# Ntropy86/review-recommender

Hardware: AMD Instinct MI355X
Metric: queries/sec at top-k=100 (hybrid alpha=0.5) (higher is better)
Workload: dtype f32; 1 GPU; hybrid BM25+dense alpha=0.5 top-k=100 pool=150, 10000000 products x 384 fp32, BM25 ~40 tokens/doc vocab 200000 (327073593 postings on rank 0, 11164874 postings per query), batches of 256 queries; query_sets=4, docs=10000000, docs_per_gpu=10000000, batch=256, k=100, pool=150, parallelism=single GPU: no collective

## Files before the change

review-recommender_amd/csrc/rr_dense.hip:

```cpp
#include <stdlib.h>

#include "rr_common.h"
#include "rr_dense.h"
#include "rr_x3.h"

#define RR_SEL_THREADS 1024
#define RR_SEL_GCAP 4096
#define RR_SEL_CCAP 12288
#define RR_SEL_SORTCAP 8192
#define RR_SEL_RCAP 8192
#define RR_SEL_LCAP 4096

template <int NF>
__device__ __forceinline__ void rr_load_rows(f32x4 (&dst)[NF], const f32x4* __restrict__ mat,
                                             int64_t row, int64_t n_rows, int sub) {
    row = row < n_rows ? row : n_rows - 1;
    const f32x4* p = mat + row * (int64_t)(NF * 16) + sub;
#pragma unroll
    for (int i = 0; i < NF; ++i) dst[i] = __builtin_nontemporal_load(p + 16 * i);
}

template <int NF, int NB, bool FROM_LDS>
__device__ __forceinline__ void rr_dot_rows(const f32x4 (&x)[NF], const f32x4 (&qreg)[NF],
                                            const f32x4 (*qs)[NF * 16], int sub, int it,
// ... 376 lines not shown
    uint32_t n_cand = counters[1];

    if (n_cand > RR_SEL_SORTCAP) {
        uint64_t prefix = 0, mask = 0;
        uint32_t k = (uint32_t)pool;
        for (int shift = 56; shift >= 0; shift -= 8) {
            if (tid < 256) hist[tid] = 0;
            __syncthreads();
            for (int64_t i = tid; i < n_slots; i += RR_SEL_THREADS) {
                const int64_t t = all_tiles ? (i >> 6) : (int64_t)glist[i >> 6];
                const int64_t row = t * 64 + (i & 63);
                if (row < n_rows) {
                    const uint64_t key = ((uint64_t)rr_f2key(score_at(row)) << 32) |
                                         (uint64_t)(0xFFFFFFFFu - (uint32_t)row);
                    if ((key & mask) == prefix) atomicAdd(&hist[(key >> shift) & 255u], 1u);
                }
            }
            __syncthreads();
            rr_pick_bin(hist, wsum, sel, k);
            prefix |= (uint64_t)sel[0] << shift;
            mask |= (uint64_t)255u << shift;
            k -= sel[1];
            __syncthreads();
        }
        if (tid == 0) counters[1] = 0;
        __syncthreads();
        for (int64_t i = tid; i < n_slots; i += RR_SEL_THREADS) {
            const int64_t t = all_tiles ? (i >> 6) : (int64_t)glist[i >> 6];
            const int64_t row = t * 64 + (i & 63);
            if (row < n_rows) {
                const uint64_t key = ((uint64_t)rr_f2key(score_at(row)) << 32) |
                                     (uint64_t)(0xFFFFFFFFu - (uint32_t)row);
                if (key >= prefix) {
                    const uint32_t slot = atomicAdd(&counters[1], 1u);
                    if (slot < RR_SEL_SORTCAP) cand[slot] = key;
                }
            }
        }
        __syncthreads();
        n_cand = counters[1] < RR_SEL_SORTCAP ? counters[1] : RR_SEL_SORTCAP;
    }

    if (n_cand > RR_SEL_SORTCAP) n_cand = RR_SEL_SORTCAP;
    int n_sort = 1;
    while (n_sort < (int)n_cand) n_sort <<= 1;
    for (int i = tid; i < n_sort; i += RR_SEL_THREADS)
        if (i >= (int)n_cand) cand[i] = 0;
    rr_bitonic_desc(cand, n_sort);
}

#define RR_SEL_RK 8
template <int RK>
__device__ uint32_t rr_kth_largest_reg(const uint32_t (&r)[RR_SEL_RK], int n_mine, uint32_t k,
                                       uint32_t (*cnt)[3][16], int& phase, int max_steps) {
    const int tid = threadIdx.x;
    const int ln = tid & 63;
    uint32_t mx = 0, mn = 0xFFFFFFFFu, nz = 0;
#pragma unroll
    for (int j = 0; j < RK; ++j) {
        const bool live = j < n_mine && r[j] != 0u;
        if (j < n_mine) mx = r[j] > mx ? r[j] : mx;
        if (live) mn = r[j] < mn ? r[j] : mn;
        nz += (uint32_t)__popcll(__ballot(live));
    }
#pragma unroll
    for (int m = 32; m >= 1; m >>= 1) {
        const uint32_t a = __shfl_xor(mx, m, 64), b = __shfl_xor(mn, m, 64);
        mx = a > mx ? a : mx;
        mn = b < mn ? b : mn;
    }
    if (ln == 0) {
        cnt[phase][0][tid >> 6] = mx;
        cnt[phase][1][tid >> 6] = mn;
        cnt[phase][2][tid >> 6] = nz;
    }
    __syncthreads();
    uint32_t nz_all = 0;
    for (int w = 0; w < 16; ++w) {
        mx = cnt[phase][0][w] > mx ? cnt[phase][0][w] : mx;
        mn = cnt[phase][1][w] < mn ? cnt[phase][1][w] : mn;
        nz_all += cnt[phase][2][w];
    }
    if (nz_all < k) mn = 0u;
    phase ^= 1;
    if (mx == mn) return mx;
    int bit = 31 - __clz(mx ^ mn);
    uint32_t prefix = (bit == 31) ? 0u : (mx >> (bit + 1)) << (bit + 1);
    for (int step = 0; bit >= 0 && step < max_steps; ++step) {
        const int lo = bit >= 1 ? bit - 1 : 0;
        const bool two = bit >= 1;
        const uint32_t t1 = prefix | (1u << lo);
        const uint32_t t2 = prefix | (1u << bit);
        const uint32_t t3 = prefix | (1u << bit) | (1u << lo);
        uint32_t c1 = 0, c2 = 0, c3 = 0;
#pragma unroll
        for (int j = 0; j < RK; ++j) {
            const bool have = j < n_mine;
            c1 += (uint32_t)__popcll(__ballot(have && r[j] >= t1));
            c2 += (uint32_t)__popcll(__ballot(have && r[j] >= t2));
            c3 += (uint32_t)__popcll(__ballot(have && r[j] >= t3));
        }
        if (ln == 0) {
            cnt[phase][0][tid >> 6] = c1;
            cnt[phase][1][tid >> 6] = c2;
            cnt[phase][2][tid >> 6] = c3;
        }
        __syncthreads();
        int v = ln < 48 ? (int)(&cnt[phase][0][0])[ln] : 0;
        v += __builtin_amdgcn_update_dpp(0, v, 0xB1, 0xF, 0xF, true);
        v += __builtin_amdgcn_update_dpp(0, v, 0x4E, 0xF, 0xF, true);
        v += __builtin_amdgcn_update_dpp(0, v, 0x141, 0xF, 0xF, true);
        v += __builtin_amdgcn_update_dpp(0, v, 0x140, 0xF, 0xF, true);
        const uint32_t s1 = (uint32_t)__builtin_amdgcn_readlane(v, 0);
        const uint32_t s2 = (uint32_t)__builtin_amdgcn_readlane(v, 16);
        const uint32_t s3 = (uint32_t)__builtin_amdgcn_readlane(v, 32);
        phase ^= 1;
        if (two) {
            if (s3 >= k) prefix = t3;
            else if (s2 >= k) prefix = t2;
            else if (s1 >= k) prefix = t1;
        } else if (s2 >= k) {
            prefix = t2;
        }
        bit = lo - 1;
    }
    return prefix;
}

__device__ void rr_rank_sort_desc(const uint64_t* keys, int n, uint64_t* out) {
    const int tid = threadIdx.x;
    uint64_t mine = 0;
    int rank = 0;
    if (tid < n) {
        mine = keys[tid];
        for (int j = 0; j < n; ++j) rank += keys[j] > mine ? 1 : 0;
    }
    __syncthreads();
    if (tid < n) out[rank] = mine;
    __syncthreads();
}

template <typename GroupKeyAt>
__device__ uint32_t rr_sel_open_groups(GroupKeyAt group_key_at, int ng, int pool, uint32_t (*cnt)[3][16],
                                       int& phase, uint32_t* counters, uint32_t* list2,
                                       float eps2 = -1.f, uint32_t* open_key = nullptr, uint32_t thr_floor = 0u) {
    const int tid = threadIdx.x;
    uint32_t r[RR_SEL_RK];
    int n_mine = 0;
#pragma unroll
    for (int j = 0; j < RR_SEL_RK; ++j) {
        const int i = tid + j * RR_SEL_THREADS;
        r[j] = i < ng ? group_key_at(i) : 0u;
        n_mine += i < ng ? 1 : 0;
    }
    uint32_t tau = 1u;
    if (ng > pool) {
        if (ng <= 1 * RR_SEL_THREADS) tau = rr_kth_largest_reg<1>(r, n_mine, (uint32_t)pool, cnt, phase, 7);
        else if (ng <= 2 * RR_SEL_THREADS) tau = rr_kth_largest_reg<2>(r, n_mine, (uint32_t)pool, cnt, phase, 7);
        else if (ng <= 4 * RR_SEL_THREADS) tau = rr_kth_largest_reg<4>(r, n_mine, (uint32_t)pool, cnt, phase, 7);
        else tau = rr_kth_largest_reg<8>(r, n_mine, (uint32_t)pool, cnt, phase, 7);
    }
    if (tau == 0u) tau = 1u;
    uint32_t thr = tau;
    if (eps2 >= 0.f) {
        thr = rr_f2key(rr_key2f(tau) - eps2);
        if (thr == 0u) thr = 1u;
        if (thr_floor > thr) thr = thr_floor;
        if (open_key) *open_key = thr;
    }
#pragma unroll
    for (int j = 0; j < RR_SEL_RK; ++j) {
        if (j < n_mine && r[j] >= thr) {
            const uint32_t slot = atomicAdd(&counters[0], 1u);
            if (slot < RR_SEL_LCAP) list2[slot] = (uint32_t)(tid + j * RR_SEL_THREADS);
        }
    }
    __syncthreads();
    return tau;
}

__global__ __launch_bounds__(RR_SEL_THREADS) void rr_select(
    rr_scan_geom G, const float* __restrict__ sims, const float* __restrict__ gmax,
    const uint32_t* __restrict__ smax, int pool, int64_t row_offset,
    int64_t* __restrict__ out_rows, float* __restrict__ out_scores, int32_t* __restrict__ dbg,
    const int32_t* __restrict__ only_if, int n_total, int64_t sims_slice, int64_t gmax_slice, int64_t smax_slice,
    const int32_t* __restrict__ qlist, int32_t* __restrict__ clear_flags) {
    if (qlist) {
        if ((int)blockIdx.x >= qlist[0]) return;
        const int qo = qlist[1 + blockIdx.x] - (int)blockIdx.x;
        out_rows += (int64_t)qo * pool; out_scores += (int64_t)qo * pool; dbg += qo * 16;
        if (threadIdx.x == 0) clear_flags[qo + (int)blockIdx.x] = 0;
    }
    if (gridDim.y > 1) {
        const int y = blockIdx.y;
        if (64 * y + (int)blockIdx.x >= n_total) return;
        only_if += 64 * y;
        out_rows += (int64_t)64 * y * pool; out_scores += (int64_t)64 * y * pool; dbg += 64 * y * 16;
        sims += y * sims_slice; gmax += y * gmax_slice; smax += y * smax_slice;
    }
    if (only_if && !only_if[blockIdx.x]) return;
    __shared__ uint32_t hist[256];
    __shared__ uint32_t wsum[4];
    __shared__ uint32_t cnt[2][3][16];
    __shared__ uint32_t sel[2];
    __shared__ uint32_t counters[4];
    __shared__ uint32_t list2[RR_SEL_LCAP];
    __shared__ uint32_t list1[RR_SEL_GCAP];
    __shared__ uint64_t cand[RR_SEL_CCAP];

    const int tid = threadIdx.x;
    const int q = blockIdx.x;
    const int QS = G.qs;
    auto score_at = [&](int64_t row) -> float {
        return QS ? sims[((row >> 4) * QS + q) * 16 + (row & 15)] : sims[(int64_t)q * G.n_pad + row];
    };
    auto tile_max_at = [&](int64_t t) -> float {
        return QS ? gmax[t * QS + q] : gmax[(int64_t)q * G.n_tiles + t];
    };
    auto group_key_at = [&](int i) -> uint32_t {
        return QS ? smax[(int64_t)i * QS + q] : smax[(int64_t)q * G.n_waves + i];
    };
    const int64_t n_rows = G.n_rows, n_tiles = G.n_tiles;
    int phase = 0;
    long long stamp[8];
    int n_stamp = 0;
#define RR_STAMP() do { if (n_stamp < 8) stamp[n_stamp++] = clock64(); } while (0)
    RR_STAMP();
    const int ng = G.n_waves;
    bool fast = ng <= RR_SEL_RK * RR_SEL_THREADS;

    if (tid < 4) counters[tid] = 0;
    __syncthreads();

    if (fast) {
        const uint32_t tau = rr_sel_open_groups(group_key_at, ng, pool, cnt, phase, counters, list2);
        RR_STAMP();
        if (counters[0] > RR_SEL_LCAP) fast = false;

        if (fast) {
            const int C = (int)G.tiles_per_wave;
            const int64_t n2 = (int64_t)counters[0] * C;
            for (int64_t i = tid; i < n2; i += RR_SEL_THREADS) {
                const int64_t t = (int64_t)list2[i / C] * C + (i % C);
                if (t < n_tiles && rr_f2key(tile_max_at(t)) >= tau) {
                    const uint32_t slot = atomicAdd(&counters[1], 1u);
                    if (slot < RR_SEL_GCAP) list1[slot] = (uint32_t)t;
                }
            }
            __syncthreads();
            if (counters[1] > RR_SEL_GCAP) fast = false;
        }
        RR_STAMP();
        if (fast) {
            const int n1 = (int)counters[1] * 64;
            for (int i = tid; i < n1; i += RR_SEL_THREADS) {
                const uint32_t row = list1[i >> 6] * 64u + (uint32_t)(i & 63);
                if ((int64_t)row < n_rows) {
                    const uint32_t key = rr_f2key(score_at(row));
                    if (key >= tau) {
                        const uint32_t slot = atomicAdd(&counters[2], 1u);
                        if (slot < RR_SEL_CCAP / 2)
                            cand[slot] = ((uint64_t)key << 32) | (uint64_t)(0xFFFFFFFFu - row);
                    }
                }
            }
            __syncthreads();
            RR_STAMP();
            const uint32_t n_cand = counters[2];
            if (n_cand > RR_SEL_CCAP / 2 || n_cand < (uint32_t)pool) {
                fast = false;
            } else if (n_cand <= RR_SEL_THREADS) {
                rr_rank_sort_desc(cand, (int)n_cand, cand + RR_SEL_CCAP / 2);
                for (int i = tid; i < pool; i += RR_SEL_THREADS) cand[i] = cand[RR_SEL_CCAP / 2 + i];
                __syncthreads();
            } else {
                int n_sort = 1;
                while (n_sort < (int)n_cand) n_sort <<= 1;
                for (int i = tid; i < n_sort; i += RR_SEL_THREADS)
                    if (i >= (int)n_cand) cand[i] = 0;
                rr_bitonic_desc(cand, n_sort);
            }
        }
    }
    RR_STAMP();
    if (tid == 0) {
        dbg[q * 16 + 0] = fast ? 1 : 0;
        dbg[q * 16 + 1] = (int32_t)counters[0];
        dbg[q * 16 + 2] = (int32_t)counters[1];
        dbg[q * 16 + 3] = (int32_t)counters[2];
        for (int i = 1; i < 8; ++i) dbg[q * 16 + 3 + i] = i < n_stamp ? (int32_t)(stamp[i] - stamp[i - 1]) : -1;
    }
    if (!fast) {
        __syncthreads();
        rr_select_slow(score_at, tile_max_at, n_rows, n_tiles, pool, hist, wsum, sel, counters, list1, cand);
    }
    for (int i = tid; i < pool; i += RR_SEL_THREADS) {
        const uint64_t key = cand[i];
        const uint32_t row = 0xFFFFFFFFu - (uint32_t)(key & 0xFFFFFFFFu);
        out_rows[(int64_t)q * pool + i] = (int64_t)row + row_offset;
        out_scores[(int64_t)q * pool + i] = rr_key2f((uint32_t)(key >> 32));
    }
}

__global__ __launch_bounds__(RR_SEL_THREADS) void rr_select_mtiles(
    rr_scan_geom G, const float* __restrict__ mmax, const uint32_t* __restrict__ smax, int pool,
    uint32_t* __restrict__ out_mtiles, int32_t* __restrict__ out_count, uint32_t* __restrict__ out_tau,
    int32_t* __restrict__ fb, int32_t* __restrict__ dbg, const float* __restrict__ eps,
    const float* __restrict__ sigma, int nq_a, int nq_b, int64_t mmax_set_stride, int64_t smax_set_stride,
    const float* __restrict__ floor) {
    __shared__ uint32_t cnt[2][3][16];
    __shared__ uint32_t counters[4];
    __shared__ uint32_t list2[RR_SEL_LCAP];
    const int tid = threadIdx.x;
    const int Q = blockIdx.x;
    const int set = (nq_b > 0 && Q >= nq_a) ? 1 : 0;
    const int q = set ? Q - nq_a : Q;
    const int nq_set = set ? nq_b : nq_a;
    mmax += set * mmax_set_stride;
    smax += set * smax_set_stride;
    if (eps) eps += set * RR_FLT_MAXQ;
    if (sigma) sigma += set * RR_FLT_MAXQ;
    out_mtiles += (int64_t)(Q - q) * RR_X3_MCAP;
    out_count += Q - q; out_tau += Q - q; fb += Q - q; dbg += (Q - q) * 16;
    const int QS = G.qs;
    auto group_key_at = [&](int i) -> uint32_t { return smax[(int64_t)i * QS + q]; };
    const int gpw = G.gpw > 1 ? G.gpw : 1;
    const int ng = G.n_waves * gpw;
    int phase = 0;
    const long long c0 = clock64();
    long long c1 = c0, c2 = c0;
    if (tid < 4) counters[tid] = 0;
    __syncthreads();
    bool ok = ng <= RR_SEL_RK * RR_SEL_THREADS && ng > pool;
    uint32_t tau = 1u;
    uint32_t open = 1u;
    if (ok) {
        const float e = eps ? eps[q] : -1.f;
        if (eps && !(e >= 0.f && e < 3.0e38f)) ok = false;
        if (ok) {
            const float fl = (floor && eps) ? floor[Q] - 1.05f * e : -INFINITY;
            if (fl > -3.0e38f) {
                open = rr_f2key(fl);
                if (open == 0u) open = 1u;
                for (int i = tid; i < ng; i += RR_SEL_THREADS) {
                    if (group_key_at(i) >= open) {
                        const uint32_t slot = atomicAdd(&counters[0], 1u);
                        if (slot < RR_SEL_LCAP) list2[slot] = (uint32_t)i;
                    }
                }
                __syncthreads();
                tau = rr_f2key(floor[Q]);
                if (counters[0] > RR_SEL_LCAP) {
                    __syncthreads();
                    if (tid == 0) counters[0] = 0;
                    __syncthreads();
                    const uint32_t floor_open = open, floor_tau = tau;
                    tau = rr_sel_open_groups(group_key_at, ng, pool, cnt, phase, counters, list2, 2.05f * e, &open, floor_open);
                    tau = rr_f2key(rr_key2f(tau) - 1.02f * e);
                    if (floor_tau > tau) tau = floor_tau;
                }
            } else {
                tau = rr_sel_open_groups(group_key_at, ng, pool, cnt, phase, counters, list2, eps ? 2.05f * e : -1.f, &open, 0u);
                if (!eps) open = tau;
                else tau = rr_f2key(rr_key2f(tau) - 1.02f * e);
            }
            if (tau == 0u) tau = 1u;
            if (counters[0] > RR_SEL_LCAP) ok = false;
        }
    }
    c1 = clock64();
    if (ok) {
        const int C = (int)G.tiles_per_group;
        const int64_t n2 = (int64_t)counters[0] * C;
        const f32x4* mm4 = reinterpret_cast<const f32x4*>(mmax);
        if (G.mm_pairs == 3) {
            constexpr int U = 4;
            const float step = rr_flt_gap_step(eps, nq_set);
            const float openf = open <= 0x007FFFFFu ? -INFINITY : rr_key2f(open);
            if (sigma && !(sigma[q] <= openf)) ok = false;
            const int n2i = (int)n2;
            for (int i0 = tid; i0 < n2i; i0 += U * RR_SEL_THREADS) {
                int64_t tt[U];
                uint32_t w0[U], w1[U];
#pragma unroll
                for (int u = 0; u < U; ++u) {
                    const int i = i0 + u * RR_SEL_THREADS;
                    tt[u] = -1;
                    if (i < n2i) {
                        const int g = (int)list2[i / C], k = g % gpw, j = i % C;
                        const int64_t in_run = (int64_t)k * C + j;
                        const int64_t t = (int64_t)(g / gpw) * G.tiles_per_wave + in_run;
                        if (in_run < G.tiles_per_wave && t < G.n_tiles) tt[u] = t;
                    }
                    const int64_t ts = tt[u] < 0 ? 0 : tt[u];
                    w0[u] = reinterpret_cast<const uint32_t*>(mmax)[(2 * ts) * QS + q];
                    w1[u] = reinterpret_cast<const uint32_t*>(mmax)[(2 * ts + 1) * QS + q];
                }
#pragma unroll
                for (int u = 0; u < U; ++u) {
                    if (tt[u] < 0) continue;
#pragma unroll
                    for (int half = 0; half < 2; ++half) {
                        const uint32_t w = half ? w1[u] : w0[u];
                        const float mx = __uint_as_float(w << 16);
                        if (!(mx >= openf)) continue;
#pragma unroll
                        for (int g = 0; g < 4; ++g) {
                            const uint32_t code = (w >> (16 + 4 * g)) & 15u;
                            const float bound = mx - rr_flt_gap_steps(code) * step;
                            if (bound >= openf) {
                                const uint32_t slot = atomicAdd(&counters[1], 1u);
                                if (slot < RR_X3_MCAP) out_mtiles[(int64_t)q * RR_X3_MCAP + slot] = (uint32_t)(tt[u] * 8 + 4 * half + g);
                            }
                        }
                    }
                }
            }
        } else
        for (int64_t i = tid; i < n2; i += RR_SEL_THREADS) {
            const int g = (int)list2[i / C], k = g % gpw, j = (int)(i % C);
            const int64_t in_run = (int64_t)k * C + j;
            const int64_t t = (int64_t)(g / gpw) * G.tiles_per_wave + in_run;
            if (in_run >= G.tiles_per_wave || t >= G.n_tiles) continue;
            float v[4];
            if (G.mm_pairs) {
                const float2 m0 = reinterpret_cast<const float2*>(mmax)[(2 * t) * QS + q];
                const float2 m1 = reinterpret_cast<const float2*>(mmax)[(2 * t + 1) * QS + q];
                v[0] = m0.x, v[1] = m0.y, v[2] = m1.x, v[3] = m1.y;
            } else {
                const f32x4 m = mm4[t * QS + q];
                v[0] = m.x, v[1] = m.y, v[2] = m.z, v[3] = m.w;
            }
#pragma unroll
            for (int sub = 0; sub < 4; ++sub) {
                if (rr_f2key(v[sub]) >= open) {
                    const uint32_t slot = atomicAdd(&counters[1], 1u);
                    if (slot < RR_X3_MCAP) out_mtiles[(int64_t)q * RR_X3_MCAP + slot] = (uint32_t)(t * 4 + sub);
                }
            }
        }
        __syncthreads();
        if (counters[1] > RR_X3_MCAP) ok = false;
    }
    c2 = clock64();
    if (tid == 0) {
        out_count[q] = ok ? (int32_t)counters[1] : 0;
        out_tau[q] = tau;
        fb[q] = ok ? 0 : 1;
        dbg[q * 16 + 0] = ok ? 2 : 0;
        dbg[q * 16 + 1] = (int32_t)counters[0];
        dbg[q * 16 + 2] = (int32_t)counters[1];
        dbg[q * 16 + 3] = 0;
        dbg[q * 16 + 4] = (int32_t)(c1 - c0);
        dbg[q * 16 + 5] = (int32_t)(c2 - c1);
        for (int i = 6; i < 16; ++i) dbg[q * 16 + i] = -1;
#ifdef RR_DEBUG_HARNESS
        dbg[q * 16 + 6] = (int32_t)open;
#endif
    }
}

template <int RCAP>
__global__ __launch_bounds__(RR_SEL_THREADS) void rr_select_rescored(
    rr_scan_geom G, const uint32_t* __restrict__ mtiles, const int32_t* __restrict__ count,
    const uint32_t* __restrict__ tau_of, const float* __restrict__ sc, int pool, int64_t row_offset,
    int64_t* __restrict__ out_rows, float* __restrict__ out_scores, int32_t* __restrict__ fb,
    int32_t* __restrict__ dbg, int floor_mode) {
    __shared__ uint32_t counters[2];
    __shared__ uint64_t cand[RCAP];
    const int tid = threadIdx.x;
    const int q = blockIdx.x;
    if (fb[q]) return;
    if (tid < 2) counters[tid] = 0;
    __syncthreads();
    const uint32_t tau = tau_of[q];
    const int sh = G.mm_pairs == 3 ? 3 : 4;
    const int n1 = count[q] << sh;
    const bool all_rows = floor_mode && (uint32_t)n1 <= RCAP / 2;
    for (int i = tid; i < n1 && !all_rows; i += RR_SEL_THREADS) {
        const int64_t at = (int64_t)q * RR_X3_MCAP + (i >> sh);
        const int r = i & ((1 << sh) - 1);
        const uint32_t row = (mtiles[at] << sh) + (uint32_t)r;
        if ((int64_t)row < G.n_rows) {
            const uint32_t key = rr_f2key(sc[(at << sh) + r]);
            if (key >= tau) {
                const uint32_t slot = atomicAdd(&counters[0], 1u);
                if (slot < RCAP / 2) cand[slot] = ((uint64_t)key << 32) | (uint64_t)(0xFFFFFFFFu - row);
            }
        }
    }
    __syncthreads();
    uint32_t n_cand = counters[0];
    if (all_rows || (floor_mode && n_cand < (uint32_t)pool && (uint32_t)n1 <= RCAP / 2)) {
        __syncthreads();
        if (tid == 0) counters[0] = 0;
        __syncthreads();
        for (int i = tid; i < n1; i += RR_SEL_THREADS) {
            const int64_t at = (int64_t)q * RR_X3_MCAP + (i >> sh);
            const int r = i & ((1 << sh) - 1);
            const uint32_t row = (mtiles[at] << sh) + (uint32_t)r;
            if ((int64_t)row < G.n_rows) {
                const uint32_t key = rr_f2key(sc[(at << sh) + r]);
                const uint32_t slot = atomicAdd(&counters[0], 1u);
                if (slot < RCAP / 2) cand[slot] = ((uint64_t)key << 32) | (uint64_t)(0xFFFFFFFFu - row);
            }
        }
        __syncthreads();
        n_cand = counters[0];
    }
    if (tid == 0) dbg[q * 16 + 3] = (int32_t)n_cand;
    if (n_cand > RCAP / 2 || n_cand < (uint32_t)pool) {
        if (tid == 0) {
            fb[q] = 1;
            dbg[q * 16 + 0] = 0;
        }
        return;
    }
    if (n_cand <= RR_SEL_THREADS) {
        rr_rank_sort_desc(cand, (int)n_cand, cand + RCAP / 2);
        for (int i = tid; i < pool; i += RR_SEL_THREADS) cand[i] = cand[RCAP / 2 + i];
        __syncthreads();
    } else {
        int n_sort = 1;
        while (n_sort < (int)n_cand) n_sort <<= 1;
        for (int i = tid; i < n_sort; i += RR_SEL_THREADS)
            if (i >= (int)n_cand) cand[i] = 0;
        rr_bitonic_desc(cand, n_sort);
    }
    for (int i = tid; i < pool; i += RR_SEL_THREADS) {
        const uint64_t key = cand[i];
        const uint32_t row = 0xFFFFFFFFu - (uint32_t)(key & 0xFFFFFFFFu);
        out_rows[(int64_t)q * pool + i] = (int64_t)row + row_offset;
        out_scores[(int64_t)q * pool + i] = rr_key2f((uint32_t)(key >> 32));
    }
}

rr_x3_scratch rr_x3_scratch_of(const rr_index* ix) {
    rr_x3_scratch s;
    char* p = static_cast<char*>(ix->d_x3);
    s.mtiles = reinterpret_cast<uint32_t*>(p);  p += sizeof(uint32_t) * RR_SEL_MAXQ * RR_X3_MCAP;
    s.count = reinterpret_cast<int32_t*>(p);    p += sizeof(int32_t) * RR_SEL_MAXQ;
    s.tau = reinterpret_cast<uint32_t*>(p);     p += sizeof(uint32_t) * RR_SEL_MAXQ;
    s.fb = reinterpret_cast<int32_t*>(p);       p += sizeof(int32_t) * RR_SEL_MAXQ;
    p += sizeof(float) * RR_SEL_MAXQ;
    s.eps = ix->d_eps;
    s.sc = reinterpret_cast<float*>(p);
    return s;
}
size_t rr_x3_scratch_bytes() {
    return sizeof(uint32_t) * RR_SEL_MAXQ * RR_X3_MCAP + 4 * sizeof(int32_t) * RR_SEL_MAXQ +
           sizeof(float) * (size_t)RR_SEL_MAXQ * RR_X3_MCAP * 16;
}
void rr_launch_select_mtiles(rr_index* ix, const rr_scan_geom& G, int nq, int pool, hipStream_t st, const float* eps,
                             const float* sigma, int nq_b, int64_t mmax_set_stride, int64_t smax_set_stride,
                             const float* floor) {
    const rr_x3_scratch s = rr_x3_scratch_of(ix);
    hipLaunchKernelGGL(rr_select_mtiles, dim3(nq + nq_b), dim3(RR_SEL_THREADS), 0, st, G, ix->d_gmax, ix->d_smax, pool,
                       s.mtiles, s.count, s.tau, s.fb, ix->d_sel_trace, eps, sigma, nq, nq_b, mmax_set_stride,
                       smax_set_stride, floor);
}
void rr_launch_select_rescored(rr_index* ix, const rr_scan_geom& G, int nq, int pool, int64_t* d_rows,
                               float* d_scores, hipStream_t st, bool floor_mode) {
    const rr_x3_scratch s = rr_x3_scratch_of(ix);
    if (pool <= 512)
        hipLaunchKernelGGL((rr_select_rescored<RR_SEL_RCAP>), dim3(nq), dim3(RR_SEL_THREADS), 0, st, G, s.mtiles, s.count, s.tau,
                           s.sc, pool, ix->row_offset, d_rows, d_scores, s.fb, ix->d_sel_trace, floor_mode ? 1 : 0);
    else
        hipLaunchKernelGGL((rr_select_rescored<RR_SEL_CCAP>), dim3(nq), dim3(RR_SEL_THREADS), 0, st, G, s.mtiles, s.count, s.tau,
                           s.sc, pool, ix->row_offset, d_rows, d_scores, s.fb, ix->d_sel_trace, floor_mode ? 1 : 0);
}

__global__ __launch_bounds__(RR_SEL_THREADS) void rr_group_kth(rr_scan_geom G, const uint32_t* __restrict__ smax, int kth,
                                                               const float* __restrict__ eps, float* __restrict__ bound,
                                                               int nq_a, int nq_b, int64_t smax_set_stride) {
    __shared__ uint32_t cnt[2][3][16];
    const int tid = threadIdx.x;
    const int Q = blockIdx.x;
    const int set = (nq_b > 0 && Q >= nq_a) ? 1 : 0;
    const int q = set ? Q - nq_a : Q;
    smax += set * smax_set_stride;
    eps += set * RR_FLT_MAXQ;
    const int QS = G.qs;
    const int gpw = G.gpw > 1 ? G.gpw : 1;
    const int ng = G.n_waves * gpw;
    int phase = 0;
    float out = -INFINITY;
    if (ng > kth && ng <= RR_SEL_RK * RR_SEL_THREADS) {
        uint32_t r[RR_SEL_RK];
        int n_mine = 0;
#pragma unroll
        for (int j = 0; j < RR_SEL_RK; ++j) {
            const int i = tid + j * RR_SEL_THREADS;
            r[j] = i < ng ? smax[(int64_t)i * QS + q] : 0u;
            n_mine += i < ng ? 1 : 0;
        }
        uint32_t tau;
        if (ng <= 1 * RR_SEL_THREADS) tau = rr_kth_largest_reg<1>(r, n_mine, (uint32_t)kth, cnt, phase, 7);
        else if (ng <= 2 * RR_SEL_THREADS) tau = rr_kth_largest_reg<2>(r, n_mine, (uint32_t)kth, cnt, phase, 7);
        else if (ng <= 4 * RR_SEL_THREADS) tau = rr_kth_largest_reg<4>(r, n_mine, (uint32_t)kth, cnt, phase, 7);
        else tau = rr_kth_largest_reg<8>(r, n_mine, (uint32_t)kth, cnt, phase, 7);
        const float e = eps[q];
        if (tau > 0x007FFFFFu && e >= 0.f && e < 3.0e38f) out = rr_key2f(tau) - 1.01f * e;
        if (!(out == out)) out = -INFINITY;
    }
    if (tid == 0) bound[Q] = out;
}
void rr_launch_group_kth(rr_index* ix, const rr_scan_geom& G, int nq_a, int nq_b, int kth, const float* eps, float* d_bound,
                         int64_t smax_set_stride, hipStream_t st) {
    hipLaunchKernelGGL(rr_group_kth, dim3(nq_a + nq_b), dim3(RR_SEL_THREADS), 0, st, G, ix->d_smax, kth, eps, d_bound, nq_a,
                       nq_b, smax_set_stride);
}

__global__ void rr_l2norm_f32(float* __restrict__ mat, int64_t n_rows, int dim_pad, float eps) {
    const int lane = threadIdx.x & 63;
    const int64_t row = (int64_t)blockIdx.x * (blockDim.x >> 6) + (threadIdx.x >> 6);
    if (row >= n_rows) return;
    float* p = mat + row * dim_pad;
    float ss = 0.f;
    for (int i = lane; i < dim_pad; i += 64) ss = __builtin_fmaf(p[i], p[i], ss);
#pragma unroll
    for (int m = 32; m >= 1; m >>= 1) ss += __shfl_xor(ss, m, 64);
    const float nrm = fmaxf(sqrtf(ss), eps);
    for (int i = lane; i < dim_pad; i += 64) p[i] = p[i] / nrm;
}

static int rr_ensure_maxima(rr_index* ix, int nq) {
    const size_t nm = nq >= RR_MFMA_MAXQ ? RR_FLT_MAXQ : nq;
    if (ix->maxima_q >= (int)nm) return RR_OK;
    const int64_t n_tiles = rr_round_up(ix->n_rows, 64) / 64;
    if (ix->d_gmax) hipFree(ix->d_gmax);
    if (ix->d_smax) hipFree(ix->d_smax);
    ix->d_gmax = nullptr;
    ix->d_smax = nullptr;
    ix->maxima_q = 0;
    const size_t groups_cap = (size_t)RR_MAX_SCAN_WAVES;
    const size_t gmax_words = nm * n_tiles * 4 + (size_t)RR_MAX_SCAN_WAVES * RR_FLT_MAXQ;
    RR_HIP_TRY(hipMalloc(&ix->d_gmax, sizeof(float) * gmax_words));
    RR_HIP_TRY(hipMemsetD32Async((hipDeviceptr_t)ix->d_gmax, 0x0000FF80, gmax_words, nullptr));
    RR_HIP_TRY(hipStreamSynchronize(nullptr));
    RR_HIP_TRY(hipMalloc(&ix->d_smax, sizeof(uint32_t) * 2 * nm * groups_cap));
    ix->maxima_q = (int32_t)nm;
    return RR_OK;
}

static int rr_ensure_scratch(rr_index* ix, int nq) {
    const int rc = rr_ensure_maxima(ix, nq);
    if (rc) return rc;
    if (ix->scratch_q >= nq || (ix->scratch_small && ix->scratch_q >= RR_MFMA_MAXQ)) return RR_OK;
    const int64_t n_tiles = rr_round_up(ix->n_rows, 64) / 64;
    if (ix->d_sims) hipFree(ix->d_sims);
    ix->d_sims = nullptr;
    ix->scratch_q = 0;
    static const bool force_small = getenv("RR_SCRATCH_SMALL") != nullptr;
    if ((force_small && nq > RR_MFMA_MAXQ) ||
        hipMalloc(&ix->d_sims, sizeof(float) * (size_t)nq * n_tiles * 64) != hipSuccess) {
        (void)hipGetLastError();
        ix->d_sims = nullptr;
        if (nq <= RR_MFMA_MAXQ) { rr_set_error("rr_dense_topk: out of device memory for the score scratch"); return RR_E_NOMEM; }
        nq = RR_MFMA_MAXQ;
        RR_HIP_TRY(hipMalloc(&ix->d_sims, sizeof(float) * (size_t)nq * n_tiles * 64));
        ix->scratch_small = true;
    }
    ix->scratch_q = nq;
    return RR_OK;
}

static void rr_slot_store(const rr_index* ix, rr_scan_slot& s) {
    s.d_q = ix->d_q; s.d_qplanes = ix->d_qplanes; s.d_eps = ix->d_eps; s.d_gmax = ix->d_gmax; s.d_smax = ix->d_smax;
    s.maxima_q = ix->maxima_q; s.d_flt_samp = ix->d_flt_samp; s.d_flt_sigma = ix->d_flt_sigma; s.d_flt_prog = ix->d_flt_prog;
    s.flt_seq = ix->flt_seq; s.flt_prep_fresh = ix->flt_prep_fresh; s.flt_pending = ix->flt_pending;
}
static void rr_slot_fetch(rr_index* ix, const rr_scan_slot& s) {
    ix->d_q = s.d_q; ix->d_qplanes = s.d_qplanes; ix->d_eps = s.d_eps; ix->d_gmax = s.d_gmax; ix->d_smax = s.d_smax;
    ix->maxima_q = s.maxima_q; ix->d_flt_samp = s.d_flt_samp; ix->d_flt_sigma = s.d_flt_sigma; ix->d_flt_prog = s.d_flt_prog;
    ix->flt_seq = s.flt_seq; ix->flt_prep_fresh = s.flt_prep_fresh; ix->flt_pending = s.flt_pending;
}
void rr_slot_park(rr_index* ix) {
    rr_slot_store(ix, ix->parked[ix->cur_slot]);
    rr_slot_fetch(ix, rr_scan_slot());
}
int rr_slot_activate(rr_index* ix, int slot) {
    RR_REQUIRE(slot >= 0 && slot < RR_SCAN_SLOTS, "scan slot %d outside [0, %d)", slot, RR_SCAN_SLOTS);
    if (slot != ix->cur_slot) {
        rr_slot_store(ix, ix->parked[ix->cur_slot]);
        rr_slot_fetch(ix, ix->parked[slot]);
        ix->parked[slot] = rr_scan_slot();
        ix->cur_slot = slot;
    }
    if (!ix->d_q) {
        RR_HIP_TRY(hipSetDevice(ix->device));
        RR_HIP_TRY(hipMalloc(&ix->d_qplanes, (size_t)2 * 3 * 64 * 384 * 2));
        RR_HIP_TRY(hipMalloc((void**)&ix->d_eps, sizeof(float) * RR_SEL_MAXQ));
        RR_HIP_TRY(hipMalloc((void**)&ix->d_q, sizeof(float) * (size_t)RR_MAX_BATCH * ix->dim_pad));
    }
    return RR_OK;
}

template <typename K>
static int rr_resident_grid(K kernel, int device) {
    int per_cu = 0, cus = 0;
    if (hipOccupancyMaxActiveBlocksPerMultiprocessor(&per_cu, kernel, RR_SCAN_THREADS, 0) != hipSuccess ||
        per_cu < 1)
        per_cu = 2;
    if (hipDeviceGetAttribute(&cus, hipDeviceAttributeMultiprocessorCount, device) != hipSuccess || cus < 1)
        cus = 256;
    int grid = per_cu * cus;
    if (grid * (RR_SCAN_THREADS / 64) > RR_MAX_SCAN_WAVES) grid = RR_MAX_SCAN_WAVES / (RR_SCAN_THREADS / 64);
    return grid;
}

rr_scan_geom rr_make_geom(const rr_index* ix, int resident_blocks) {
    rr_scan_geom G;
    G.n_rows = ix->n_rows;
    G.n_tiles = rr_round_up(ix->n_rows, 64) / 64;
    G.n_pad = G.n_tiles * 64;
    int64_t max_waves = (int64_t)resident_blocks * (RR_SCAN_THREADS / 64);
    if (ix->scan_cus > 0 && ix->n_cus > 0) {
        max_waves = max_waves * ix->scan_cus / ix->n_cus;
        if (max_waves < 1) max_waves = 1;
    }
    G.tiles_per_wave = (G.n_tiles + max_waves - 1) / max_waves;
    G.n_waves = (int32_t)((G.n_tiles + G.tiles_per_wave - 1) / G.tiles_per_wave);
    G.qs = 0;
    G.mm_pairs = 0;
    G.gpw = 1;
    G.tiles_per_group = G.tiles_per_wave;
    return G;
}

int rr_scan_events_begin(rr_index* ix, hipStream_t st) {
    const int slot = (int)(ix->ring_head % rr_index::kRing);
    hipEventRecord(ix->ring0[slot], st);
    return slot;
}
void rr_scan_events_end(rr_index* ix, int slot, hipStream_t st) {
    hipEventRecord(ix->ring1[slot], st);
    ix->ring_head++;
    if (ix->ring_head - ix->ring_tail > rr_index::kRing) ix->ring_tail = ix->ring_head - rr_index::kRing;
}
void rr_launch_select(rr_index* ix, const rr_scan_geom& G, int nq, int pool, int64_t* d_rows,
                      float* d_scores, hipStream_t st, const int32_t* only_if, int slices, int64_t sims_slice,
                      int64_t gmax_slice, int64_t smax_slice) {
    const dim3 grid(slices > 1 ? RR_MFMA_MAXQ : nq, slices > 1 ? slices : 1);
    hipLaunchKernelGGL(rr_select, grid, dim3(RR_SEL_THREADS), 0, st, G, ix->d_sims, ix->d_gmax,
                       ix->d_smax, pool, ix->row_offset, d_rows, d_scores, ix->d_sel_trace, only_if, nq, sims_slice,
                       gmax_slice, smax_slice, (const int32_t*)nullptr, (int32_t*)nullptr);
}
int rr_resident_waves(const void* kernel, int threads, int device) {
    int per_cu = 0, cus = 0;
    if (hipOccupancyMaxActiveBlocksPerMultiprocessor(&per_cu, kernel, threads, 0) != hipSuccess || per_cu < 1)
        per_cu = 1;
    if (hipDeviceGetAttribute(&cus, hipDeviceAttributeMultiprocessorCount, device) != hipSuccess || cus < 1)
        cus = 256;
    int waves = per_cu * cus * (threads / 64);
    return waves > RR_MAX_SCAN_WAVES ? RR_MAX_SCAN_WAVES : waves;
}

template <int NB>
static rr_scan_geom rr_launch_scan(rr_index* ix, const float* d_q, hipStream_t st) {
    const f32x4* mat = reinterpret_cast<const f32x4*>(ix->d_matrix);
    const int nf = ix->dim_pad / 64;
    static int cap6 = 0, capg = 0;
    rr_scan_geom G;
    if (nf == 6) {
        if (!cap6) cap6 = rr_resident_grid(rr_scan_f32<6, NB>, ix->device);
        G = rr_make_geom(ix, cap6);
        const int grid = (G.n_waves + 3) / 4;
        hipLaunchKernelGGL((rr_scan_f32<6, NB>), dim3(grid), dim3(RR_SCAN_THREADS), 0, st, mat, G, d_q,
                           ix->d_sims, ix->d_gmax, ix->d_smax, (const int32_t*)nullptr, 0, (int32_t*)nullptr);
    } else {
        if (!capg) capg = rr_resident_grid(rr_scan_f32_generic<NB>, ix->device);
        G = rr_make_geom(ix, capg);
        const int grid = (G.n_waves + 3) / 4;
        hipLaunchKernelGGL((rr_scan_f32_generic<NB>), dim3(grid), dim3(RR_SCAN_THREADS), 0, st, mat, G, nf,
                           d_q, ix->d_sims, ix->d_gmax, ix->d_smax);
    }
    return G;
}

int rr_dense_listed_fallback(rr_index* ix, const float* d_q, int nq, int pool, int64_t* d_rows, float* d_scores,
                             int32_t* flags, hipStream_t st) {
    static const bool off = getenv("RR_NO_CHAIN_FALLBACK") != nullptr;
    if (off || ix->dtype != RR_DTYPE_F32 || ix->dim_pad != 384 || !ix->d_flag_list) return RR_OK;
    static int cap = 0;
    if (!cap) cap = rr_resident_grid(rr_scan_f32<6, 8, true>, ix->device);
    rr_scan_geom G = rr_make_geom(ix, cap);
    hipLaunchKernelGGL((rr_scan_f32<6, 8, true>), dim3((G.n_waves + 3) / 4), dim3(RR_SCAN_THREADS), 0, st,
                       reinterpret_cast<const f32x4*>(ix->d_matrix), G, d_q, ix->d_sims, ix->d_gmax, ix->d_smax,
                       (const int32_t*)flags, nq, ix->d_flag_list);
    hipLaunchKernelGGL(rr_select, dim3(8), dim3(RR_SEL_THREADS), 0, st, G, ix->d_sims, ix->d_gmax, ix->d_smax, pool,
                       ix->row_offset, d_rows, d_scores, ix->d_sel_trace, (const int32_t*)nullptr, 8, (int64_t)0, (int64_t)0,
                       (int64_t)0, (const int32_t*)ix->d_flag_list, flags);
    RR_HIP_TRY(hipGetLastError());
    return RR_OK;
}

static int rr_dense_chunk(rr_index* ix, const float* d_q, int nq, int pool, int64_t* d_rows,
                          float* d_scores, hipStream_t st, bool time_it) {
    if (time_it) hipEventRecord(ix->ev0, st);
    const int slot = (int)(ix->ring_head % rr_index::kRing);
    hipEventRecord(ix->ring0[slot], st);
    rr_scan_note(ix, 1, nq <= 1 ? 1 : nq <= 2 ? 2 : nq <= 4 ? 4 : 8, nq, 0);
    rr_scan_geom G;
    switch (nq) {
        case 1: G = rr_launch_scan<1>(ix, d_q, st); break;
        case 2: G = rr_launch_scan<2>(ix, d_q, st); break;
        case 3: case 4: G = rr_launch_scan<4>(ix, d_q, st); break;
        default: G = rr_launch_scan<8>(ix, d_q, st); break;
    }
    hipEventRecord(ix->ring1[slot], st);
    ix->ring_head++;
    if (ix->ring_head - ix->ring_tail > rr_index::kRing) ix->ring_tail = ix->ring_head - rr_index::kRing;
    if (time_it) {
        hipEventRecord(ix->ev1, st);
        ix->timing_valid = true;
    }
    hipLaunchKernelGGL(rr_select, dim3(nq), dim3(RR_SEL_THREADS), 0, st, G, ix->d_sims, ix->d_gmax,
                       ix->d_smax, pool, ix->row_offset, d_rows, d_scores, ix->d_sel_trace, (const int32_t*)nullptr, nq, (int64_t)0, (int64_t)0, (int64_t)0,
                       (const int32_t*)nullptr, (int32_t*)nullptr);
    RR_HIP_TRY(hipGetLastError());
    return RR_OK;
}

template <int NQT>
static int rr_dense_chunk_mfma(rr_index* ix, const float* d_q, int nq, int pool, int64_t* d_rows,
                               float* d_scores, hipStream_t st) {
    constexpr int THREADS = NQT == 4 ? 512 : 256;
    static int cap_waves = 0;
    if (!cap_waves) {
        int per_cu = 0, cus = 0;
        if (hipOccupancyMaxActiveBlocksPerMultiprocessor(&per_cu, rr_scan_mfma_f32<NQT>, THREADS, 0) != hipSuccess ||
            per_cu < 1)
            per_cu = 1;
        if (hipDeviceGetAttribute(&cus, hipDeviceAttributeMultiprocessorCount, ix->device) != hipSuccess || cus < 1)
            cus = 256;
        cap_waves = per_cu * cus * (THREADS / 64);
        if (cap_waves > RR_MAX_SCAN_WAVES) cap_waves = RR_MAX_SCAN_WAVES;
    }
    rr_scan_geom G = rr_make_geom(ix, cap_waves / 4);
    G.qs = 16 * NQT;
    const int slot = (int)(ix->ring_head % rr_index::kRing);
    hipEventRecord(ix->ring0[slot], st);
    rr_scan_note(ix, 6, NQT, nq, 0);
    hipLaunchKernelGGL((rr_scan_mfma_f32<NQT>), dim3((G.n_waves + THREADS / 64 - 1) / (THREADS / 64)), dim3(THREADS), 0, st,
                       reinterpret_cast<const f32x4*>(ix->d_matrix), G, d_q, ix->d_sims, ix->d_gmax, ix->d_smax);
    hipEventRecord(ix->ring1[slot], st);
    ix->ring_head++;
    if (ix->ring_head - ix->ring_tail > rr_index::kRing) ix->ring_tail = ix->ring_head - rr_index::kRing;
    hipLaunchKernelGGL(rr_select, dim3(nq), dim3(RR_SEL_THREADS), 0, st, G, ix->d_sims, ix->d_gmax,
                       ix->d_smax, pool, ix->row_offset, d_rows, d_scores, ix->d_sel_trace, (const int32_t*)nullptr, nq, (int64_t)0, (int64_t)0, (int64_t)0,
                       (const int32_t*)nullptr, (int32_t*)nullptr);
    RR_HIP_TRY(hipGetLastError());
    return RR_OK;
}

static int rr_scratch_enter(rr_index* ix, hipStream_t st, bool scan = true, bool select = true) {
    (void)scan;
    const int s = ix->cur_slot;
    if (ix->slot_has[s] && ix->slot_stream[s] != st) RR_HIP_TRY(hipStreamWaitEvent(st, ix->slot_ev[s], 0));
    if (select && ix->has_done && st != ix->last_stream) RR_HIP_TRY(hipStreamWaitEvent(st, ix->ev_done, 0));
    return RR_OK;
}
// ... 324 lines not shown
```

Baseline: 136,900 queries/s.

## Split mtile selection into threshold and multi-block list kernels with transposed keys

Factors the threshold search out of rr_select_mtiles into a helper. Selection now runs as three kernels: a transpose of the per-group max keys into per-query contiguous rows, a per-query threshold kernel that writes its open-group list to global scratch, and a list kernel that spreads each query's tile scan over several blocks. The list kernel stages survivors in LDS and merges them through global atomics and a ticket counter. The aim is to remove the strided key reads and the single-block serial scan per query, at the cost of two extra launches, more scratch memory, and cross-block atomics.

```diff
diff --git a/review-recommender_amd/csrc/rr_dense.hip b/review-recommender_amd/csrc/rr_dense.hip
--- a/review-recommender_amd/csrc/rr_dense.hip
+++ b/review-recommender_amd/csrc/rr_dense.hip
@@ -702,38 +702,15 @@
     }
 }
 
-__global__ __launch_bounds__(RR_SEL_THREADS) void rr_select_mtiles(
-    rr_scan_geom G, const float* __restrict__ mmax, const uint32_t* __restrict__ smax, int pool,
-    uint32_t* __restrict__ out_mtiles, int32_t* __restrict__ out_count, uint32_t* __restrict__ out_tau,
-    int32_t* __restrict__ fb, int32_t* __restrict__ dbg, const float* __restrict__ eps,
-    const float* __restrict__ sigma, int nq_a, int nq_b, int64_t mmax_set_stride, int64_t smax_set_stride,
-    const float* __restrict__ floor) {
-    __shared__ uint32_t cnt[2][3][16];
-    __shared__ uint32_t counters[4];
-    __shared__ uint32_t list2[RR_SEL_LCAP];
+
+template <typename GroupKeyAt>
+__device__ bool rr_sel_mtiles_threshold(GroupKeyAt group_key_at, int ng, int pool, const float* __restrict__ eps,
+                                        const float* __restrict__ floor, int q, int Q, uint32_t (*cnt)[3][16], int& phase,
+                                        uint32_t* counters, uint32_t* list2, uint32_t& tau, uint32_t& open) {
     const int tid = threadIdx.x;
-    const int Q = blockIdx.x;
-    const int set = (nq_b > 0 && Q >= nq_a) ? 1 : 0;
-    const int q = set ? Q - nq_a : Q;
-    const int nq_set = set ? nq_b : nq_a;
-    mmax += set * mmax_set_stride;
-    smax += set * smax_set_stride;
-    if (eps) eps += set * RR_FLT_MAXQ;
-    if (sigma) sigma += set * RR_FLT_MAXQ;
-    out_mtiles += (int64_t)(Q - q) * RR_X3_MCAP;
-    out_count += Q - q; out_tau += Q - q; fb += Q - q; dbg += (Q - q) * 16;
-    const int QS = G.qs;
-    auto group_key_at = [&](int i) -> uint32_t { return smax[(int64_t)i * QS + q]; };
-    const int gpw = G.gpw > 1 ? G.gpw : 1;
-    const int ng = G.n_waves * gpw;
-    int phase = 0;
-    const long long c0 = clock64();
-    long long c1 = c0, c2 = c0;
-    if (tid < 4) counters[tid] = 0;
-    __syncthreads();
     bool ok = ng <= RR_SEL_RK * RR_SEL_THREADS && ng > pool;
-    uint32_t tau = 1u;
-    uint32_t open = 1u;
+    tau = 1u;
+    open = 1u;
     if (ok) {
         const float e = eps ? eps[q] : -1.f;
         if (eps && !(e >= 0.f && e < 3.0e38f)) ok = false;
@@ -768,6 +745,41 @@
             if (counters[0] > RR_SEL_LCAP) ok = false;
         }
     }
+    return ok;
+}
+
+__global__ __launch_bounds__(RR_SEL_THREADS) void rr_select_mtiles(
+    rr_scan_geom G, const float* __restrict__ mmax, const uint32_t* __restrict__ smax, int pool,
+    uint32_t* __restrict__ out_mtiles, int32_t* __restrict__ out_count, uint32_t* __restrict__ out_tau,
+    int32_t* __restrict__ fb, int32_t* __restrict__ dbg, const float* __restrict__ eps,
+    const float* __restrict__ sigma, int nq_a, int nq_b, int64_t mmax_set_stride, int64_t smax_set_stride,
+    const float* __restrict__ floor) {
+    __shared__ uint32_t cnt[2][3][16];
+    __shared__ uint32_t counters[4];
+    __shared__ uint32_t list2[RR_SEL_LCAP];
+    const int tid = threadIdx.x;
+    const int Q = blockIdx.x;
+    const int set = (nq_b > 0 && Q >= nq_a) ? 1 : 0;
+    const int q = set ? Q - nq_a : Q;
+    const int nq_set = set ? nq_b : nq_a;
+    mmax += set * mmax_set_stride;
+    smax += set * smax_set_stride;
+    if (eps) eps += set * RR_FLT_MAXQ;
+    if (sigma) sigma += set * RR_FLT_MAXQ;
+    out_mtiles += (int64_t)(Q - q) * RR_X3_MCAP;
+    out_count += Q - q; out_tau += Q - q; fb += Q - q; dbg += (Q - q) * 16;
+    const int QS = G.qs;
+    auto group_key_at = [&](int i) -> uint32_t { return smax[(int64_t)i * QS + q]; };
+    const int gpw = G.gpw > 1 ? G.gpw : 1;
+    const int ng = G.n_waves * gpw;
+    int phase = 0;
+    const long long c0 = clock64();
+    long long c1 = c0, c2 = c0;
+    if (tid < 4) counters[tid] = 0;
+    __syncthreads();
+    uint32_t tau = 1u;
+    uint32_t open = 1u;
+    bool ok = rr_sel_mtiles_threshold(group_key_at, ng, pool, eps, floor, q, Q, cnt, phase, counters, list2, tau, open);
     c1 = clock64();
     if (ok) {
         const int C = (int)G.tiles_per_group;
@@ -860,6 +872,179 @@
     }
 }
 
+struct rr_sel_split {
+    uint32_t* keys_t;
+    uint32_t* groups;
+    int32_t* n_groups;
+    uint32_t* total;
+    uint32_t* ticket;
+    uint32_t* open;
+};
+#define RR_SEL_KEYS_T (RR_SEL_RK * RR_SEL_THREADS)
+#define RR_SEL_LIST_THREADS 256
+#define RR_SEL_LIST_STAGE 1024
+
+__global__ __launch_bounds__(256) void rr_sel_transpose_keys(const uint32_t* __restrict__ smax, uint32_t* __restrict__ keys_t, int ng,
+                                                             int QS, int nq_a, int nq_b, int64_t smax_set_stride) {
+    __shared__ uint32_t t[64][RR_FLT_MAXQ + 1];
+    const int set = blockIdx.y, nq_set = set ? nq_b : nq_a, g0 = blockIdx.x * 64;
+    smax += set * smax_set_stride;
+    keys_t += (size_t)set * RR_FLT_MAXQ * RR_SEL_KEYS_T;
+    for (int e = threadIdx.x; e < 64 * QS; e += 256) {
+        const int r = e / QS, c = e % QS;
+        if (c < nq_set && g0 + r < ng) t[r][c] = smax[(int64_t)(g0 + r) * QS + c];
+    }
+    __syncthreads();
+    for (int e = threadIdx.x; e < 64 * nq_set; e += 256) {
+        const int c = e >> 6, r = e & 63;
+        if (g0 + r < ng) keys_t[(size_t)c * RR_SEL_KEYS_T + g0 + r] = t[r][c];
+    }
+}
+
+__global__ __launch_bounds__(RR_SEL_THREADS) void rr_select_mtiles_threshold(
+    rr_scan_geom G, const uint32_t* __restrict__ smax, int pool, int32_t* __restrict__ out_count, uint32_t* __restrict__ out_tau,
+    int32_t* __restrict__ fb, int32_t* __restrict__ dbg, const float* __restrict__ eps, const float* __restrict__ sigma, int nq_a,
+    int nq_b, int64_t smax_set_stride, const float* __restrict__ floor, rr_sel_split S, int keys_transposed) {
+    __shared__ uint32_t cnt[2][3][16];
+    __shared__ uint32_t counters[4];
+    __shared__ uint32_t list2[RR_SEL_LCAP];
+    const int tid = threadIdx.x;
+    const int Q = blockIdx.x;
+    const int set = (nq_b > 0 && Q >= nq_a) ? 1 : 0;
+    const int q = set ? Q - nq_a : Q;
+    smax += set * smax_set_stride;
+    if (eps) eps += set * RR_FLT_MAXQ;
+    if (sigma) sigma += set * RR_FLT_MAXQ;
+    const int QS = G.qs;
+    const uint32_t* __restrict__ mine = S.keys_t + (size_t)(set * RR_FLT_MAXQ + q) * RR_SEL_KEYS_T;
+    auto group_key_at = [&](int i) -> uint32_t { return keys_transposed ? mine[i] : smax[(int64_t)i * QS + q]; };
+    const int gpw = G.gpw > 1 ? G.gpw : 1;
+    const int ng = G.n_waves * gpw;
+    int phase = 0;
+    const long long c0 = clock64();
+    if (tid < 4) counters[tid] = 0;
+    __syncthreads();
+    uint32_t tau = 1u, open = 1u;
+    const bool ok = rr_sel_mtiles_threshold(group_key_at, ng, pool, eps, floor, q, Q, cnt, phase, counters, list2, tau, open);
+    const uint32_t n_open = counters[0];
+    if (ok)
+        for (uint32_t i = tid; i < n_open; i += RR_SEL_THREADS) S.groups[(size_t)Q * RR_SEL_LCAP + i] = list2[i];
+    if (tid == 0) {
+        const float openf = open <= 0x007FFFFFu ? -INFINITY : rr_key2f(open);
+        const bool up = !ok || (sigma && !(sigma[q] <= openf));
+        S.n_groups[Q] = ok ? (int32_t)n_open : -1;
+        S.total[Q] = 0u;
+        S.ticket[Q] = 0u;
+        S.open[Q] = open;
+        out_count[Q] = 0;
+        out_tau[Q] = tau;
+        fb[Q] = up ? 1 : 0;
+        dbg[Q * 16 + 0] = up ? 0 : 2;
+        dbg[Q * 16 + 1] = (int32_t)n_open;
+        dbg[Q * 16 + 2] = 0;
+        dbg[Q * 16 + 3] = 0;
+        dbg[Q * 16 + 4] = (int32_t)(clock64() - c0);
+        dbg[Q * 16 + 5] = 0;
+        for (int i = 6; i < 16; ++i) dbg[Q * 16 + i] = -1;
+#ifdef RR_DEBUG_HARNESS
+        dbg[Q * 16 + 6] = (int32_t)open;
+#endif
+    }
+}
+
+__global__ __launch_bounds__(RR_SEL_LIST_THREADS) void rr_select_mtiles_list(
+    rr_scan_geom G, const float* __restrict__ mmax, uint32_t* __restrict__ out_mtiles, int32_t* __restrict__ out_count,
+    int32_t* __restrict__ fb, int32_t* __restrict__ dbg, const float* __restrict__ eps, int nq_a, int nq_b,
+    int64_t mmax_set_stride, rr_sel_split S) {
+    __shared__ uint32_t stage[RR_SEL_LIST_STAGE];
+    __shared__ uint32_t n_stage, base;
+    const int tid = threadIdx.x;
+    const int Q = blockIdx.y;
+    const int n_open = S.n_groups[Q];
+    if (n_open < 0) return;
+    const long long c1 = clock64();
+    const int set = (nq_b > 0 && Q >= nq_a) ? 1 : 0;
+    const int q = set ? Q - nq_a : Q;
+    const int nq_set = set ? nq_b : nq_a;
+    const uint32_t* __restrict__ words = reinterpret_cast<const uint32_t*>(mmax) + set * mmax_set_stride;
+    const uint32_t* __restrict__ list2 = S.groups + (size_t)Q * RR_SEL_LCAP;
+    out_mtiles += (int64_t)Q * RR_X3_MCAP;
+    eps += set * RR_FLT_MAXQ;
+    const int QS = G.qs;
+    const int gpw = G.gpw > 1 ? G.gpw : 1;
+    if (tid == 0) n_stage = 0u;
+    __syncthreads();
+    const int C = (int)G.tiles_per_group;
+    const int n2 = n_open * C;
+    const int per = (n2 + (int)gridDim.x - 1) / (int)gridDim.x;
+    const int lo = (int)blockIdx.x * per, hi = lo + per < n2 ? lo + per : n2;
+    constexpr int U = 4;
+    const float step = rr_flt_gap_step(eps, nq_set);
+    const uint32_t open = S.open[Q];
+    const float openf = open <= 0x007FFFFFu ? -INFINITY : rr_key2f(open);
+    for (int i0 = lo + tid; i0 < hi; i0 += U * RR_SEL_LIST_THREADS) {
+        int64_t tt[U];
+        uint32_t w0[U], w1[U];
+#pragma unroll
+        for (int u = 0; u < U; ++u) {
+            const int i = i0 + u * RR_SEL_LIST_THREADS;
+            tt[u] = -1;
+            if (i < hi) {
+                const int g = (int)list2[i / C], k = g % gpw, j = i % C;
+                const int64_t in_run = (int64_t)k * C + j;
+                const int64_t t = (int64_t)(g / gpw) * G.tiles_per_wave + in_run;
+                if (in_run < G.tiles_per_wave && t < G.n_tiles) tt[u] = t;
+            }
+            const int64_t ts = tt[u] < 0 ? 0 : tt[u];
+            w0[u] = words[(2 * ts) * QS + q];
+            w1[u] = words[(2 * ts + 1) * QS + q];
+        }
+#pragma unroll
+        for (int u = 0; u < U; ++u) {
+            if (tt[u] < 0) continue;
+#pragma unroll
+            for (int half = 0; half < 2; ++half) {
+                const uint32_t w = half ? w1[u] : w0[u];
+                const float mx = __uint_as_float(w << 16);
+                if (!(mx >= openf)) continue;
+#pragma unroll
+                for (int g = 0; g < 4; ++g) {
+                    const uint32_t code = (w >> (16 + 4 * g)) & 15u;
+                    const float bound = mx - rr_flt_gap_steps(code) * step;
+                    if (bound >= openf) {
+                        const uint32_t id = (uint32_t)(tt[u] * 8 + 4 * half + g);
+                        const uint32_t slot = atomicAdd(&n_stage, 1u);
+                        if (slot < RR_SEL_LIST_STAGE) {
+                            stage[slot] = id;
+                        } else {
+                            const uint32_t at = atomicAdd(&S.total[Q], 1u);
+                            if (at < RR_X3_MCAP) out_mtiles[at] = id;
+                        }
+                    }
+                }
+            }
+        }
+    }
+    __syncthreads();
+    const uint32_t n = n_stage < RR_SEL_LIST_STAGE ? n_stage : RR_SEL_LIST_STAGE;
+    if (tid == 0) base = n ? atomicAdd(&S.total[Q], n) : 0u;
+    __syncthreads();
+    for (uint32_t i = tid; i < n; i += RR_SEL_LIST_THREADS)
+        if (base + i < RR_X3_MCAP) out_mtiles[base + i] = stage[i];
+    if (tid == 0) {
+        const uint32_t done = __hip_atomic_fetch_add(&S.ticket[Q], 1u, __ATOMIC_ACQ_REL, __HIP_MEMORY_SCOPE_AGENT);
+        if (done == gridDim.x - 1) {
+            const uint32_t total = __hip_atomic_load(&S.total[Q], __ATOMIC_ACQUIRE, __HIP_MEMORY_SCOPE_AGENT);
+            const bool up = fb[Q] != 0 || total > RR_X3_MCAP;
+            out_count[Q] = up ? 0 : (int32_t)total;
+            fb[Q] = up ? 1 : 0;
+            dbg[Q * 16 + 0] = up ? 0 : 2;
+            dbg[Q * 16 + 2] = (int32_t)total;
+            dbg[Q * 16 + 5] = (int32_t)(clock64() - c1);
+        }
+    }
+}
+
 template <int RCAP>
 __global__ __launch_bounds__(RR_SEL_THREADS) void rr_select_rescored(
     rr_scan_geom G, const uint32_t* __restrict__ mtiles, const int32_t* __restrict__ count,
@@ -947,17 +1132,44 @@
     s.sc = reinterpret_cast<float*>(p);
     return s;
 }
+static rr_sel_split rr_sel_split_of(const rr_index* ix) {
+    rr_sel_split s;
+    char* p = reinterpret_cast<char*>(rr_x3_scratch_of(ix).sc + (size_t)RR_SEL_MAXQ * RR_X3_MCAP * 16);
+    s.keys_t = reinterpret_cast<uint32_t*>(p);   p += sizeof(uint32_t) * 2 * RR_FLT_MAXQ * RR_SEL_KEYS_T;
+    s.groups = reinterpret_cast<uint32_t*>(p);   p += sizeof(uint32_t) * RR_SEL_MAXQ * RR_SEL_LCAP;
+    s.n_groups = reinterpret_cast<int32_t*>(p);  p += sizeof(int32_t) * RR_SEL_MAXQ;
+    s.total = reinterpret_cast<uint32_t*>(p);    p += sizeof(uint32_t) * RR_SEL_MAXQ;
+    s.ticket = reinterpret_cast<uint32_t*>(p);   p += sizeof(uint32_t) * RR_SEL_MAXQ;
+    s.open = reinterpret_cast<uint32_t*>(p);
+    return s;
+}
 size_t rr_x3_scratch_bytes() {
     return sizeof(uint32_t) * RR_SEL_MAXQ * RR_X3_MCAP + 4 * sizeof(int32_t) * RR_SEL_MAXQ +
-           sizeof(float) * (size_t)RR_SEL_MAXQ * RR_X3_MCAP * 16;
+           sizeof(float) * (size_t)RR_SEL_MAXQ * RR_X3_MCAP * 16 +
+           sizeof(uint32_t) * ((size_t)2 * RR_FLT_MAXQ * RR_SEL_KEYS_T + (size_t)RR_SEL_MAXQ * RR_SEL_LCAP + 4 * RR_SEL_MAXQ);
 }
 void rr_launch_select_mtiles(rr_index* ix, const rr_scan_geom& G, int nq, int pool, hipStream_t st, const float* eps,
                              const float* sigma, int nq_b, int64_t mmax_set_stride, int64_t smax_set_stride,
                              const float* floor) {
     const rr_x3_scratch s = rr_x3_scratch_of(ix);
-    hipLaunchKernelGGL(rr_select_mtiles, dim3(nq + nq_b), dim3(RR_SEL_THREADS), 0, st, G, ix->d_gmax, ix->d_smax, pool,
-                       s.mtiles, s.count, s.tau, s.fb, ix->d_sel_trace, eps, sigma, nq, nq_b, mmax_set_stride,
-                       smax_set_stride, floor);
+    static const bool no_split = getenv("RR_NO_SELECT_SPLIT") != nullptr;
+    if (no_split || G.mm_pairs != 3 || !eps || G.qs > RR_FLT_MAXQ) {
+        hipLaunchKernelGGL(rr_select_mtiles, dim3(nq + nq_b), dim3(RR_SEL_THREADS), 0, st, G, ix->d_gmax, ix->d_smax, pool,
+                           s.mtiles, s.count, s.tau, s.fb, ix->d_sel_trace, eps, sigma, nq, nq_b, mmax_set_stride,
+                           smax_set_stride, floor);
+        return;
+    }
+    const rr_sel_split S = rr_sel_split_of(ix);
+    const int ng = G.n_waves * (G.gpw > 1 ? G.gpw : 1);
+    const bool keys = ng <= RR_SEL_KEYS_T && ng > pool;
+    if (keys)
+        hipLaunchKernelGGL(rr_sel_transpose_keys, dim3((ng + 63) / 64, nq_b > 0 ? 2 : 1), dim3(256), 0, st, ix->d_smax, S.keys_t, ng,
+                           (int)G.qs, nq, nq_b, smax_set_stride);
+    hipLaunchKernelGGL(rr_select_mtiles_threshold, dim3(nq + nq_b), dim3(RR_SEL_THREADS), 0, st, G, ix->d_smax, pool, s.count, s.tau,
+                       s.fb, ix->d_sel_trace, eps, sigma, nq, nq_b, smax_set_stride, floor, S, keys ? 1 : 0);
+    static const int slices = getenv("RR_SELECT_SLICES") ? atoi(getenv("RR_SELECT_SLICES")) : 16;
+    hipLaunchKernelGGL(rr_select_mtiles_list, dim3(slices < 1 ? 1 : slices > 64 ? 64 : slices, nq + nq_b), dim3(RR_SEL_LIST_THREADS),
+                       0, st, G, ix->d_gmax, s.mtiles, s.count, s.fb, ix->d_sel_trace, eps, nq, nq_b, mmax_set_stride, S);
 }
 void rr_launch_select_rescored(rr_index* ix, const rr_scan_geom& G, int nq, int pool, int64_t* d_rows,
                                float* d_scores, hipStream_t st, bool floor_mode) {
```

Result: slower. 122,200 queries/s (-10.8%).
